# brunothg/sfm-mvs-pipeline

Measured on AMD Instinct MI355X. Metric: descriptor-pairs/s matched, higher is better.
Workload: dtype int8->int32 (exact; f32 in/out); 1 GPU; 50 images x 8192 SIFT-128 f32, unordered all-pairs (1225 pairs); descriptors_per_image=8192, pairs=1225, parallelism=pair-sharded x1

## Files before the change

sfm-mvs-pipeline_amd/csrc/match_kernels.hip:

```cpp
#include <hip/hip_runtime.h>
#include <cstdint>
#include <climits>
#include <cstdlib>
#include "match_common.hpp"
#include "diag.hpp"
#include "sift_fp6.hpp"

namespace sfmx {

typedef int i32x4 __attribute__((ext_vector_type(4)));
typedef int i32x16 __attribute__((ext_vector_type(16)));
typedef unsigned u32x4 __attribute__((ext_vector_type(4)));
typedef int i32x8 __attribute__((ext_vector_type(8)));
typedef float f32x4 __attribute__((ext_vector_type(4)));
typedef float f32x16 __attribute__((ext_vector_type(16)));

#define GLOBAL_AS __attribute__((address_space(1)))
#define LDS_AS __attribute__((address_space(3)))

__device__ __forceinline__ int med3i(int a, int b, int c) { return max(min(a, b), min(max(a, b), c)); }
__device__ __forceinline__ int v_med3(int a, int b, int c) {
    int d;
    asm("v_med3_i32 %0, %1, %2, %3" : "=v"(d) : "v"(a), "v"(b), "v"(c));
    return d;
// ... 688 lines not shown
template <bool CERT>
__device__ __forceinline__ void screen6_forward(float k1, float k2, int r1, int qi, int nt, int2 q2, int emax2, int amax2,
                                                double ratio, int pair, int64_t dense_base, int32_t* __restrict__ qlist,
                                                int32_t* __restrict__ qcount, int32_t* __restrict__ qmask,
                                                unsigned long long* __restrict__ top2, int32_t* __restrict__ qlist2,
                                                int32_t* __restrict__ qcount2) {
    const int usable = (int)(nt >= 2) & (int)(k2 > fp6::KEY_VALID);
    const int rej = usable & fp6::certainly_rejected(k1, k2, q2.x, q2.y, emax2, amax2, ratio);
    if (rej == 0) {
        const int64_t slot = dense_base + atomicAdd(&qcount[pair], 1);
        qlist[slot] = qi;
        if constexpr (CERT) {
            const int cert = fp6::certified(k1, k2, r1, nt, q2.x, q2.y, emax2, amax2, ratio);
            qmask[slot] = cert ? 1 << r1 : QMASK_FULL_ROUTE;
            if (!cert) qlist2[dense_base + atomicAdd(&qcount2[pair], 1)] = (int32_t)(slot - dense_base);
        } else {
            qmask[slot] = 0xFFFF;
        }
        top2[2 * slot] = ~0ull;
        top2[2 * slot + 1] = ~0ull;
    }
}

template <int QT, int WAVES, int MINW, int STAGE, bool CERT>
__global__ __launch_bounds__(WAVES * 64, MINW)
void sift_screen6_kernel(const WorkItem* __restrict__ work, const PairDev* __restrict__ pairs,
                         const ImgDev* __restrict__ imgs, const uint32_t* __restrict__ desc6,
                         const float* __restrict__ keyf, const int2* __restrict__ ne,
                         const int32_t* __restrict__ imax,
                         int32_t* __restrict__ qlist, int32_t* __restrict__ qcount, double ratio,
                         int32_t* __restrict__ qmask, unsigned long long* __restrict__ top2,
                         int32_t* __restrict__ qlist2, int32_t* __restrict__ qcount2) {
    static_assert(QT * WAVES * 16 == 512, "work items are 512 queries");
    static_assert(WAVES == 4 && STAGE % 128 == 0 && ROW_ALIGN % STAGE == 0, "whole DMA instructions per wave; stages inside the padded rows");
    constexpr int A_BYTES = STAGE * 64, B_BYTES = STAGE * 32;
    constexpr int GA = A_BYTES / (WAVES * 64 * 16), GB = B_BYTES / (WAVES * 64 * 16), GK = STAGE / 64;
    constexpr int BUF_BYTES = A_BYTES + B_BYTES + STAGE * 4;
    __shared__ __attribute__((aligned(16))) char lds[2 * BUF_BYTES];

    const int wid = threadIdx.x >> 6, lane = threadIdx.x & 63, g = lane >> 4, l16 = lane & 15;
    const WorkItem w = work[xcd_remap(blockIdx.x, gridDim.x)];
    const PairDev P = pairs[w.pair];
    const ImgDev L = imgs[P.left], R = imgs[P.right];
    const int nq = L.rows, nt = R.rows;
    const int qbase = w.q0 + wid * (QT * 16);

    i32x8 bq[QT];
#pragma unroll
    for (int qt = 0; qt < QT; ++qt) {
        const uint32_t* src = desc6 + (L.row0 + qbase + qt * 16 + l16) * fp6::ROW_WORDS;
        const i32x4 lo = *reinterpret_cast<const i32x4*>(src + 4 * g);
        const int2 hi = *reinterpret_cast<const int2*>(src + 16 + 2 * g);
        bq[qt] = i32x8{lo.x, lo.y, lo.z, lo.w, hi.x, hi.y, 0, 0};
    }
    float ch[QT][4];
#pragma unroll
    for (int qt = 0; qt < QT; ++qt)
#pragma unroll
        for (int i = 0; i < 4; ++i) ch[qt][i] = fp6::KEY_INIT;

    const int nstages = (nt + STAGE - 1) / STAGE;
    const char* tbase = reinterpret_cast<const char*>(desc6 + R.row0 * fp6::ROW_WORDS);
    const float* kbase = keyf + R.row0;
    auto stage = [&](int s, int buf) {
        char* base = lds + buf * BUF_BYTES;
#pragma unroll
        for (int i = 0; i < GA; ++i) {
            const int p = i * WAVES * 64 + threadIdx.x;
            const int rr = p >> 2, c = (p & 3) ^ fp6::swz_a(rr);
            const char* gp = tbase + (int64_t)(s * STAGE + rr) * fp6::ROW_BYTES + 16 * c;
            __builtin_amdgcn_global_load_lds((const GLOBAL_AS void*)gp,
                                             (LDS_AS void*)(base + (i * WAVES + wid) * 1024), 16, 0, 0);
        }
#pragma unroll
        for (int i = 0; i < GB; ++i) {
            const int p = i * WAVES * 64 + threadIdx.x;
            const int rr = p >> 1, c = (p & 1) ^ fp6::swz_b(rr);
            const char* gp = tbase + (int64_t)(s * STAGE + rr) * fp6::ROW_BYTES + 64 + 16 * c;
            __builtin_amdgcn_global_load_lds((const GLOBAL_AS void*)gp,
                                             (LDS_AS void*)(base + A_BYTES + (i * WAVES + wid) * 1024), 16, 0, 0);
        }
        if (wid < GK)
            __builtin_amdgcn_global_load_lds((const GLOBAL_AS void*)(kbase + s * STAGE + wid * 64 + lane),
                                             (LDS_AS void*)(base + A_BYTES + B_BYTES + wid * 256), 4, 0, 0);
    };

    if (nstages > 0) stage(0, 0);
    asm volatile("s_waitcnt vmcnt(0)" ::: "memory");
    __syncthreads();
    for (int s = 0; s < nstages; ++s) {
        const int buf = s & 1;
        if (s + 1 < nstages) stage(s + 1, buf ^ 1);
        const char* base = lds + buf * BUF_BYTES;
#pragma unroll
        for (int t = 0; t < STAGE / 32; ++t) {
            i32x8 a[2];
            f32x4 cinit[2];
#pragma unroll
            for (int b = 0; b < 2; ++b) {
                const int row = t * 32 + b * 16 + l16;
                const i32x4 lo = *reinterpret_cast<const i32x4*>(base + row * 64 + 16 * (g ^ fp6::swz_a(row)));
                const int2 hi = *reinterpret_cast<const int2*>(base + A_BYTES + row * 32 +
                                                               16 * ((g >> 1) ^ fp6::swz_b(row)) + 8 * (g & 1));
                a[b] = i32x8{lo.x, lo.y, lo.z, lo.w, hi.x, hi.y, 0, 0};
                cinit[b] = *reinterpret_cast<const f32x4*>(base + A_BYTES + B_BYTES + 4 * (t * 32 + b * 16 + 4 * g));
            }
#pragma unroll
            for (int qt = 0; qt < QT; ++qt) {
                const f32x4 acc0 = __builtin_amdgcn_mfma_scale_f32_16x16x128_f8f6f4(a[0], bq[qt], cinit[0], 2, 2, 0, 0x7f7f7f7f,
                                                                                    0, 0x7f7f7f7f);
                const f32x4 acc1 = __builtin_amdgcn_mfma_scale_f32_16x16x128_f8f6f4(a[1], bq[qt], cinit[1], 2, 2, 0, 0x7f7f7f7f,
                                                                                    0, 0x7f7f7f7f);
#pragma unroll
                for (int i = 0; i < 4; ++i) ch[qt][i] = fmaxf(fmaxf(ch[qt][i], acc0[i]), acc1[i]);
            }
        }
        asm volatile("s_waitcnt vmcnt(0)" ::: "memory");
        __syncthreads();
    }

    const int emax2 = imax[2 * P.right], amax2 = imax[2 * P.right + 1];
    static_assert(QT % 4 == 0, "four tiles per decision pass");
    float kk1[4] = {}, kk2[4] = {};
    int rr1[4] = {};
#pragma unroll
    for (int qt = 0; qt < QT; ++qt) {
        float k1 = fp6::KEY_INIT, k2 = fp6::KEY_INIT;
        int r1 = 4 * g;
#pragma unroll
        for (int i = 0; i < 4; ++i) {
            const float v = ch[qt][i];
            if constexpr (CERT) r1 = v > k1 ? 4 * g + i : r1;
            k2 = fmaxf(k2, fminf(k1, v));
            k1 = fmaxf(k1, v);
        }
// ... 14 lines not shown
        for (int j = 1; j < 4; ++j) {
            k1 = g == j ? kk1[j] : k1;
            k2 = g == j ? kk2[j] : k2;
            r1 = g == j ? rr1[j] : r1;
        }
        const int qi = qbase + ((qt & ~3) + g) * 16 + l16;
        if (qi >= nq || nt == 0) continue;
        screen6_forward<CERT>(k1, k2, r1, qi, nt, ne[L.row0 + qi], emax2, amax2, ratio, w.pair, P.dense_base, qlist, qcount,
                              qmask, top2, qlist2, qcount2);
    }
}

template <int WAVES, int MINW, int STAGE, bool CERT>
__global__ __launch_bounds__(WAVES * 64, MINW)
void sift_screen6w_kernel(const WorkItem* __restrict__ work, const PairDev* __restrict__ pairs,
                          const ImgDev* __restrict__ imgs, const uint32_t* __restrict__ desc6,
                          const float* __restrict__ keyf, const int2* __restrict__ ne,
                          const int32_t* __restrict__ imax,
                          int32_t* __restrict__ qlist, int32_t* __restrict__ qcount, double ratio,
                          int32_t* __restrict__ qmask, unsigned long long* __restrict__ top2,
                          int32_t* __restrict__ qlist2, int32_t* __restrict__ qcount2) {
    constexpr int QT = 4;
    static_assert(QT * WAVES * 32 == 512, "work items are 512 queries");
    static_assert(WAVES == 4 && STAGE % 128 == 0 && ROW_ALIGN % STAGE == 0, "whole DMA instructions per wave; stages inside the padded rows");
    constexpr int A_BYTES = STAGE * 64, B_BYTES = STAGE * 32;
    constexpr int GA = A_BYTES / (WAVES * 64 * 16), GB = B_BYTES / (WAVES * 64 * 16), GK = STAGE / 64;
    constexpr int BUF_BYTES = A_BYTES + B_BYTES + STAGE * 4;
    __shared__ __attribute__((aligned(16))) char lds[2 * BUF_BYTES];

    const int wid = threadIdx.x >> 6, lane = threadIdx.x & 63, h = lane >> 5, l32 = lane & 31;
    const WorkItem w = work[xcd_remap(blockIdx.x, gridDim.x)];
    const PairDev P = pairs[w.pair];
    const ImgDev L = imgs[P.left], R = imgs[P.right];
    const int nq = L.rows, nt = R.rows;
    const int qbase = w.q0 + wid * (QT * 32);

    i32x8 bq[QT][2];
#pragma unroll
    for (int qt = 0; qt < QT; ++qt) {
        const uint32_t* src = desc6 + (L.row0 + qbase + qt * 32 + l32) * fp6::ROW_WORDS;
#pragma unroll
        for (int m = 0; m < 2; ++m) {
            const int f = fp6::frag32(m, h);
            const i32x4 lo = *reinterpret_cast<const i32x4*>(src + fp6::word_index(f, 0));
            const int2 hi = *reinterpret_cast<const int2*>(src + fp6::word_index(f, 4));
            bq[qt][m] = i32x8{lo.x, lo.y, lo.z, lo.w, hi.x, hi.y, 0, 0};
        }
    }
    float ch[QT][8];
#pragma unroll
    for (int qt = 0; qt < QT; ++qt)
#pragma unroll
        for (int c = 0; c < 8; ++c) ch[qt][c] = fp6::KEY_INIT;

    const int nstages = (nt + STAGE - 1) / STAGE;
    const char* tbase = reinterpret_cast<const char*>(desc6 + R.row0 * fp6::ROW_WORDS);
    const float* kbase = keyf + R.row0;
    auto stage = [&](int s, int buf) {
        char* base = lds + buf * BUF_BYTES;
#pragma unroll
        for (int i = 0; i < GA; ++i) {
            const int p = i * WAVES * 64 + threadIdx.x;
            const int rr = p >> 2, c = (p & 3) ^ fp6::swz_a(rr);
            const char* gp = tbase + (int64_t)(s * STAGE + rr) * fp6::ROW_BYTES + 16 * c;
            __builtin_amdgcn_global_load_lds((const GLOBAL_AS void*)gp,
                                             (LDS_AS void*)(base + (i * WAVES + wid) * 1024), 16, 0, 0);
        }
#pragma unroll
        for (int i = 0; i < GB; ++i) {
            const int p = i * WAVES * 64 + threadIdx.x;
            const int rr = p >> 1, c = (p & 1) ^ fp6::swz_b(rr);
            const char* gp = tbase + (int64_t)(s * STAGE + rr) * fp6::ROW_BYTES + 64 + 16 * c;
            __builtin_amdgcn_global_load_lds((const GLOBAL_AS void*)gp,
                                             (LDS_AS void*)(base + A_BYTES + (i * WAVES + wid) * 1024), 16, 0, 0);
        }
        if (wid < GK)
            __builtin_amdgcn_global_load_lds((const GLOBAL_AS void*)(kbase + s * STAGE + wid * 64 + lane),
                                             (LDS_AS void*)(base + A_BYTES + B_BYTES + wid * 256), 4, 0, 0);
    };

    if (nstages > 0) stage(0, 0);
    asm volatile("s_waitcnt vmcnt(0)" ::: "memory");
    __syncthreads();
    for (int s = 0; s < nstages; ++s) {
        const int buf = s & 1;
        if (s + 1 < nstages) stage(s + 1, buf ^ 1);
        const char* base = lds + buf * BUF_BYTES;
#pragma unroll
        for (int t = 0; t < STAGE / 32; ++t) {
            i32x8 a[2];
            f32x16 key;
#pragma unroll
            for (int m = 0; m < 2; ++m) {
                const int f = fp6::frag32(m, h), row = t * 32 + l32;
                const i32x4 lo = *reinterpret_cast<const i32x4*>(base + fp6::lds_a32(row, f));
                const int2 hi = *reinterpret_cast<const int2*>(base + fp6::lds_b32(STAGE, row, f));
                a[m] = i32x8{lo.x, lo.y, lo.z, lo.w, hi.x, hi.y, 0, 0};
            }
#pragma unroll
            for (int k = 0; k < 4; ++k) {
                const f32x4 kv = *reinterpret_cast<const f32x4*>(base + fp6::lds_key32(STAGE, t * 32, k, h));
                key[4 * k + 0] = kv.x; key[4 * k + 1] = kv.y; key[4 * k + 2] = kv.z; key[4 * k + 3] = kv.w;
            }
#pragma unroll
            for (int qt = 0; qt < QT; ++qt) {
                f32x16 acc = __builtin_amdgcn_mfma_scale_f32_32x32x64_f8f6f4(a[0], bq[qt][0], key, 2, 2, 0, 0x7f7f7f7f, 0,
                                                                             0x7f7f7f7f);
                acc = __builtin_amdgcn_mfma_scale_f32_32x32x64_f8f6f4(a[1], bq[qt][1], acc, 2, 2, 0, 0x7f7f7f7f, 0, 0x7f7f7f7f);
#pragma unroll
                for (int c = 0; c < 8; ++c) ch[qt][c] = fmaxf(fmaxf(ch[qt][c], acc[c]), acc[c + 8]);
            }
        }
        asm volatile("s_waitcnt vmcnt(0)" ::: "memory");
        __syncthreads();
    }

    const int emax2 = imax[2 * P.right], amax2 = imax[2 * P.right + 1];
    float kk1[2] = {}, kk2[2] = {};
    int rr1[2] = {};
#pragma unroll
    for (int qt = 0; qt < QT; ++qt) {
        float k1 = fp6::KEY_INIT, k2 = fp6::KEY_INIT;
        int r1 = fp6::chain_subset32(0, h);
#pragma unroll
        for (int c = 0; c < 8; ++c) {
            const float v = ch[qt][c];
            if constexpr (CERT) r1 = v > k1 ? fp6::chain_subset32(c, h) : r1;
            k2 = fmaxf(k2, fminf(k1, v));
            k1 = fmaxf(k1, v);
        }
        {
// ... 215 lines not shown
}
#endif
hipError_t launch_prep_l2_batch(const PrepImg* tab, int n, int max_rows_pad, int8_t* desc8, int32_t* norm,
                                int32_t* keyc, int32_t* keyc2, int32_t* flags, uint32_t* desc6, float* keyf,
                                int2* ne, int32_t* imax, hipStream_t st) {
    if (n == 0 || max_rows_pad == 0) return hipSuccess;
    prep_l2_batch_kernel<<<dim3((unsigned)((max_rows_pad + PREP_ROWS - 1) / PREP_ROWS), (unsigned)n), 256, 0, st>>>(
        tab, desc8, norm, keyc, keyc2, flags, Fp6Rows{desc6, keyf, ne}, imax);
    return hipGetLastError();
}
__global__ __launch_bounds__(256)
void publish_flags_kernel(const int32_t* __restrict__ flags, int n, int32_t* __restrict__ dst, unsigned* __restrict__ seq,
                          unsigned v) {
    for (int i = threadIdx.x; i < n; i += blockDim.x) dst[i] = flags[i];
    __threadfence_system();
    __syncthreads();
    if (threadIdx.x == 0) __hip_atomic_store(seq, v, __ATOMIC_RELEASE, __HIP_MEMORY_SCOPE_SYSTEM);
}
hipError_t launch_publish_flags(const int32_t* flags, int n, int32_t* dst, unsigned* seq, unsigned v, hipStream_t st) {
    publish_flags_kernel<<<1, 256, 0, st>>>(flags, n, dst, seq, v);
    return hipGetLastError();
}
#ifdef SFMX_DIAG
hipError_t launch_probe_xor80(int8_t* p, int64_t bytes, hipStream_t st) {
    const int64_t n = bytes / 4;
    if (n == 0) return hipSuccess;
    probe_xor80_kernel<<<(unsigned)((n + 255) / 256), 256, 0, st>>>(reinterpret_cast<uint32_t*>(p), n);
    return hipGetLastError();
}
#endif

template <int ISH>
__global__ __launch_bounds__(1024)
void compact_work_kernel(const int32_t* __restrict__ porder, int n_pairs, const int32_t* __restrict__ qcount,
                         WorkItem* __restrict__ work2, int32_t* __restrict__ work2_n, int ride = 0) {
    __shared__ int wsum[16];
    const int tid = threadIdx.x, lane = tid & 63, wv = tid >> 6;
    const int per = (n_pairs + 1023) / 1024, p0 = min(tid * per, n_pairs), p1 = min(p0 + per, n_pairs);
    int mine = 0;
    auto items = [&](int c) { return c > ride ? (c + (1 << ISH) - 1) >> ISH : 0; };
    for (int i = p0; i < p1; ++i) mine += items(qcount[porder[i]]);
    int incl = mine;
    for (int o = 1; o < 64; o <<= 1) {
        const int v = __shfl_up(incl, o);
        if (lane >= o) incl += v;
    }
// ... 180 lines not shown

    for (int s = 0; s < nstages; ++s) {
        const int buf = s & 1;
        if (s + 1 < nstages) stage(s + 1, buf ^ 1);
        const char* base = lds + buf * BUF_BYTES;
#pragma unroll
        for (int t = 0; t < STAGE / 32; ++t) {
            const int row = t * 32 + l32;
            i32x4 a[4];
#pragma unroll
            for (int m = 0; m < 4; ++m) {
                const int slot = (2 * m + h) ^ ((row >> 1) & 7);
                a[m] = *reinterpret_cast<const i32x4*>(base + row * ROWB + 16 * slot);
            }
            f32x16 cinit;
#pragma unroll
            for (int g = 0; g < 4; ++g) {
                const f32x4 kv = *reinterpret_cast<const f32x4*>(base + DESC_BYTES + 4 * (t * 32 + 8 * g + 4 * h));
                cinit[4 * g + 0] = kv.x; cinit[4 * g + 1] = kv.y; cinit[4 * g + 2] = kv.z; cinit[4 * g + 3] = kv.w;
            }
            f32x16 acc[QT];
#pragma unroll
            for (int qt = 0; qt < QT; ++qt) {
                acc[qt] = __builtin_amdgcn_mfma_scale_f32_32x32x64_f8f6f4(i8of(a[0]), i8of(bq[qt][0]), cinit, 4, 4, 0,
                                                                          0x7f7f7f7f, 0, 0x7f7f7f7f);
#pragma unroll
                for (int m = 1; m < 4; ++m)
                    acc[qt] = __builtin_amdgcn_mfma_scale_f32_32x32x64_f8f6f4(i8of(a[m]), i8of(bq[qt][m]), acc[qt], 4, 4,
                                                                              0, 0x7f7f7f7f, 0, 0x7f7f7f7f);
            }
#pragma unroll
            for (int qt = 0; qt < QT; ++qt) select(acc[qt], c1[qt], c2[qt]);
        }
        if ((s % SPC) == SPC - 1 || s + 1 == nstages) {
            const int cb = (s / SPC) * CHUNK;
#pragma unroll
            for (int qt = 0; qt < QT; ++qt) {
                const float p1 = __shfl_xor(c1[qt], 32), p2 = __shfl_xor(c2[qt], 32);
                const float m1 = fmaxf(c1[qt], p1), m2 = fmaxf(fminf(c1[qt], p1), fmaxf(c2[qt], p2));
#pragma unroll
                for (int e = 0; e < 2; ++e) {
                    const float v = e == 0 ? m1 : m2;
                    if (v >= KEY_FLOOR) {
                        const float ip = __builtin_floorf(v);
                        const int dot = (int)ip - 767;
                        const int t_ = (256 - dot) >> 1;
                        const int j_ = cb + 16383 - (int)((v - ip) * 16384.0f);
                        if (t_ < T2[qt]) {
                            if (t_ < T1[qt]) { T2[qt] = T1[qt]; J2[qt] = J1[qt]; T1[qt] = t_; J1[qt] = j_; }
                            else { T2[qt] = t_; J2[qt] = j_; }
                        }
                    }
// ... 94 lines not shown
    for (int s = 0; s < nstages; ++s) {
        const int buf = s & 1;
        if (s + 1 < nstages) stage(s + 1, buf ^ 1);
        const char* base = lds + buf * BUF_BYTES;
#pragma unroll
        for (int t = 0; t < STAGE / 32; ++t) {
            i32x4 a[2][2];
            f32x4 cinit[2];
#pragma unroll
            for (int b = 0; b < 2; ++b) {
                const int row = t * 32 + b * 16 + l16;
#pragma unroll
                for (int m = 0; m < 2; ++m) {
                    const int slot = (4 * m + g) ^ ((row >> 1) & 7);
                    a[b][m] = *reinterpret_cast<const i32x4*>(base + row * ROWB + 16 * slot);
                }
                cinit[b] = *reinterpret_cast<const f32x4*>(base + DESC_BYTES + 4 * (t * 32 + b * 16 + 4 * g));
            }
#pragma unroll
            for (int qt = 0; qt < QT; ++qt) {
                f32x4 acc[2];
#pragma unroll
                for (int b = 0; b < 2; ++b) {
                    acc[b] = __builtin_amdgcn_mfma_scale_f32_16x16x128_f8f6f4(i8of(a[b][0]), i8of(bq[qt][0]), cinit[b], 4, 4,
                                                                              0, 0x7f7f7f7f, 0, 0x7f7f7f7f);
                    acc[b] = __builtin_amdgcn_mfma_scale_f32_16x16x128_f8f6f4(i8of(a[b][1]), i8of(bq[qt][1]), acc[b], 4, 4,
                                                                              0, 0x7f7f7f7f, 0, 0x7f7f7f7f);
                }
#pragma unroll
                for (int b = 0; b < 2; ++b)
#pragma unroll
                    for (int r = 0; r < 4; r += 2) {
                        const float ka = acc[b][r], kb = acc[b][r + 1];
                        c2[qt] = fmaxf(__builtin_amdgcn_fmed3f(c1[qt], ka, kb), c2[qt]);
                        c1[qt] = fmaxf(c1[qt], fmaxf(ka, kb));
                    }
            }
        }
        if ((s % SPC) == SPC - 1 || s + 1 == nstages) {
            const int cb = (s / SPC) * CHUNK;
#pragma unroll
            for (int qt = 0; qt < QT; ++qt) {
                float m1 = c1[qt], m2 = c2[qt];
#pragma unroll
                for (int o = 16; o <= 32; o <<= 1) {
                    const float p1 = __shfl_xor(m1, o), p2 = __shfl_xor(m2, o);
                    m2 = fmaxf(fminf(m1, p1), fmaxf(m2, p2));
                    m1 = fmaxf(m1, p1);
                }
#pragma unroll
// ... 103 lines not shown
    for (int s = 0; s < nstages; ++s) {
        const int buf = s & 1;
        if (s + 1 < nstages) stage(s + 1, buf ^ 1);
        const char* base = lds + buf * BUF_BYTES;
#pragma unroll
        for (int t = 0; t < STAGE / 32; ++t) {
            i32x4 a[2][2];
            f32x4 cinit[2];
#pragma unroll
            for (int b = 0; b < 2; ++b) {
                const int row = t * 32 + b * 16 + l16;
#pragma unroll
                for (int m = 0; m < 2; ++m) {
                    const int slot = (4 * m + g) ^ ((row >> 1) & 7);
                    a[b][m] = *reinterpret_cast<const i32x4*>(base + row * ROWB + 16 * slot);
                }
                cinit[b] = *reinterpret_cast<const f32x4*>(base + DESC_BYTES + 4 * (t * 32 + b * 16 + 4 * g));
            }
#pragma unroll
            for (int qt = 0; qt < QT; ++qt) {
                f32x4 acc[2];
#pragma unroll
                for (int b = 0; b < 2; ++b) {
                    acc[b] = __builtin_amdgcn_mfma_scale_f32_16x16x128_f8f6f4(i8of(a[b][0]), i8of(bq[qt][0]), cinit[b], 4, 4,
                                                                              0, 0x7f7f7f7f, 0, 0x7f7f7f7f);
                    acc[b] = __builtin_amdgcn_mfma_scale_f32_16x16x128_f8f6f4(i8of(a[b][1]), i8of(bq[qt][1]), acc[b], 4, 4,
                                                                              0, 0x7f7f7f7f, 0, 0x7f7f7f7f);
                }
#pragma unroll
                for (int i = 0; i < 4; ++i) ch[qt][i] = fmaxf(fmaxf(ch[qt][i], acc[0][i]), acc[1][i]);
            }
        }
        asm volatile("s_waitcnt vmcnt(0)" ::: "memory");
        __syncthreads();
    }

#pragma unroll
    for (int qt = 0; qt < QT; ++qt) {
        float k1 = 0.f, k2 = 0.f;
#pragma unroll
        for (int i = 0; i < 4; ++i) {
            const float v = ch[qt][i];
            k2 = fmaxf(k2, fminf(k1, v));
            k1 = fmaxf(k1, v);
        }
#pragma unroll
        for (int o = 16; o <= 32; o <<= 1) {
            const float p1 = __shfl_xor(k1, o), p2 = __shfl_xor(k2, o);
            k2 = fmaxf(fminf(k1, p1), fmaxf(k2, p2));
            k1 = fmaxf(k1, p1);
// ... 107 lines not shown
                    keys_lds[i] = (i < rows && j < nt) ? (float)(767 * 16384 + 16383 - li) * (1.0f / 16384.0f) : 0.f;
                }
                asm volatile("s_waitcnt vmcnt(0)" ::: "memory");
                __syncthreads();
                if (active) {
                    for (int t = 0; t < rows / 32; ++t) {
                        i32x4 a[2][2];
                        f32x4 cinit[2];
#pragma unroll
                        for (int b = 0; b < 2; ++b) {
                            const int row = t * 32 + b * 16 + l16;
#pragma unroll
                            for (int m = 0; m < 2; ++m) {
                                const int slot = (4 * m + g) ^ ((row >> 1) & 7);
                                a[b][m] = *reinterpret_cast<const i32x4*>(rows_lds + row * ROWB + 16 * slot);
                            }
                            cinit[b] = *reinterpret_cast<const f32x4*>(keys_lds + t * 32 + b * 16 + 4 * g);
                        }
#pragma unroll
                        for (int qt = 0; qt < QT; ++qt) {
                            f32x4 acc[2];
#pragma unroll
                            for (int b = 0; b < 2; ++b) {
                                acc[b] = __builtin_amdgcn_mfma_scale_f32_16x16x128_f8f6f4(i8of(a[b][0]), i8of(bq[qt][0]), cinit[b],
                                                                                          4, 4, 0, 0x7f7f7f7f, 0, 0x7f7f7f7f);
                                acc[b] = __builtin_amdgcn_mfma_scale_f32_16x16x128_f8f6f4(i8of(a[b][1]), i8of(bq[qt][1]), acc[b],
                                                                                          4, 4, 0, 0x7f7f7f7f, 0, 0x7f7f7f7f);
                            }
#pragma unroll
                            for (int b = 0; b < 2; ++b)
#pragma unroll
                                for (int q = 0; q < 4; q += 2) {
                                    const float ka = acc[b][q], kb = acc[b][q + 1];
                                    c2[qt] = fmaxf(__builtin_amdgcn_fmed3f(c1[qt], ka, kb), c2[qt]);
                                    c1[qt] = fmaxf(c1[qt], fmaxf(ka, kb));
                                }
                        }
                    }
                }
            }
            if (active) {
#pragma unroll
                for (int qt = 0; qt < QT; ++qt) {
                    float m1 = c1[qt], m2 = c2[qt];
#pragma unroll
                    for (int o = 16; o <= 32; o <<= 1) {
                        const float p1 = __shfl_xor(m1, o), p2 = __shfl_xor(m2, o);
                        m2 = fmaxf(fminf(m1, p1), fmaxf(m2, p2));
                        m1 = fmaxf(m1, p1);
                    }
// ... 786 lines not shown
```

sfm-mvs-pipeline_amd/csrc/matcher.cpp:

```cpp
#include <hip/hip_runtime.h>
#include "diag.hpp"
#include <algorithm>
#include <atomic>
#include <cstdio>
#include <cstdlib>
#include <cstring>
#include <mutex>
#include <numeric>
#include <string>
#include <thread>
#include <vector>

#include "../../include/sfmx.h"
#include "match_common.hpp"
#include "sift_fp6.hpp"

namespace sfmx {
hipError_t launch_prep_l2(const float*, int, int, int, int8_t*, int32_t*, int32_t*, int32_t*, int32_t*, hipStream_t);
hipError_t launch_probe_xor80(int8_t*, int64_t, hipStream_t);
hipError_t launch_publish_flags(const int32_t*, int, int32_t*, unsigned*, unsigned, hipStream_t);
hipError_t launch_prep_l2_batch(const PrepImg*, int, int, int8_t*, int32_t*, int32_t*, int32_t*, int32_t*, uint32_t*, float*,
                                int2*, int32_t*, hipStream_t);
hipError_t launch_prep_f32(const float*, int, int, int, float*, hipStream_t);
hipError_t launch_prep_hamming(const uint8_t*, int, int, int, uint8_t*, hipStream_t);
hipError_t launch_sift_knn2(const WorkItem*, int, const PairDev*, const ImgDev*, const int8_t*, const int32_t*,
                            const int32_t*, const int32_t*, int32_t*, int32_t*, int, const int32_t*, WorkItem*,
                            int32_t*, int32_t*, float*, int2*, int32_t*, double, hipStream_t, hipEvent_t, int32_t*,
                            unsigned long long*, unsigned long long*, bool, const uint32_t*, const float*, const int2*,
                            const int32_t*);
hipError_t launch_finish_lists(const PairRec*, int, const int32_t*, const int32_t*, const int32_t*, unsigned long long*,
                               const unsigned long long*, int2*, int32_t*, const int8_t*, const int32_t*, const int32_t*,
                               const float*, double, int, int, int, int, int64_t*, int32_t*, int64_t*, DMatchDev*, int32_t*,
                               hipStream_t, hipEvent_t);
bool persist_screens();
hipError_t launch_sift_slow(const int2*, const int32_t*, const PairDev*, const ImgDev*, const int8_t*,
                            const int32_t*, int32_t*, float*, double, hipStream_t);
hipError_t launch_sift_f32(const WorkItem*, int, const PairDev*, const ImgDev*, const float*, int32_t*, float*,
                           double, hipStream_t);
hipError_t launch_orb_knn2(const WorkItem*, int, const PairDev*, const ImgDev*, const uint8_t*, int32_t*, float*,
                           double, hipStream_t);
hipError_t launch_prep_hamming_fp4(const uint8_t*, int, int, int, uint8_t*, int32_t*, hipStream_t);
hipError_t launch_orb_mfma(const WorkItem*, int, const PairDev*, const ImgDev*, const uint8_t*, const int32_t*,
// ... 759 lines not shown
    for (int p = 0; p < m->n_pairs; ++p) { a += h[p]; b += h[arena_qcount2(m->n_pairs) + p]; }
    if (forwarded) *forwarded = a;
    if (full_route) *full_route = b;
    return SFMX_OK;
}
int sfmx_diag_matcher_prep_rows(sfmx_matcher* m, int img, uint32_t* desc6, float* keyf, int32_t* ne, int32_t* norm,
                                int32_t* imax) {
    if (!m) return fail(SFMX_EINVAL, "null matcher");
    if (m->norm != SFMX_NORM_L2 || img < 0 || img >= m->n_imgs) return fail(SFMX_EINVAL, "no such L2 image");
    DeviceGuard g(m->device);
    if (hipDeviceSynchronize() != hipSuccess) return fail(SFMX_EINTERNAL, "device synchronize failed");
    const ImgDev& d = m->imgs[img];
    const size_t n = (size_t)d.rows_pad;
    hipError_t e = hipSuccess;
    if (desc6 && e == hipSuccess)
        e = hipMemcpy(desc6, m->desc6.as<uint32_t>() + d.row0 * fp6::ROW_WORDS, n * fp6::ROW_BYTES, hipMemcpyDeviceToHost);
    if (keyf && e == hipSuccess) e = hipMemcpy(keyf, m->keyf.as<float>() + d.row0, n * 4, hipMemcpyDeviceToHost);
    if (ne && e == hipSuccess) e = hipMemcpy(ne, m->ne.as<int2>() + d.row0, n * sizeof(int2), hipMemcpyDeviceToHost);
    if (norm && e == hipSuccess) e = hipMemcpy(norm, m->normv.as<int32_t>() + d.row0, n * 4, hipMemcpyDeviceToHost);
    if (imax && e == hipSuccess) e = hipMemcpy(imax, m->imax.as<int32_t>() + 2 * img, 8, hipMemcpyDeviceToHost);
    if (e != hipSuccess) return fail(SFMX_EINTERNAL, hipGetErrorString(e));
    return d.rows_pad;
}
#endif

int sfmx_matcher_timing(sfmx_matcher* m, float* main_kernel_ms, float* total_ms) {
    if (!m) return fail(SFMX_EINVAL, "null matcher");
    if (!m->ev_recorded) return fail(SFMX_ESTATE, "no timing before run");
    DeviceGuard g(m->device);
    HIPCHK(hipEventSynchronize(m->ev[2]));
    float a = 0.f, b = 0.f;
    HIPCHK(hipEventElapsedTime(&a, m->ev[0], m->ev[1]));
    HIPCHK(hipEventElapsedTime(&b, m->ev[0], m->ev[2]));
    if (main_kernel_ms) *main_kernel_ms = a;
    if (total_ms) *total_ms = b;
    return SFMX_OK;
}

int sfmx_matcher_timing_history(sfmx_matcher* m, float* main_kernel_ms, float* screen_ms, int32_t n) {
    if (!m) return fail(SFMX_EINVAL, "null matcher");
    if (!m->ev_recorded) return fail(SFMX_ESTATE, "no timing before run");
    if (n < 0) return fail(SFMX_EINVAL, "negative count");
    DeviceGuard g(m->device);
    HIPCHK(hipEventSynchronize(m->ev[2]));
    const long long k = std::min<long long>({(long long)n, m->runs, (long long)sfmx_matcher::EV_RING});
    for (long long i = 0; i < k; ++i) {
// ... 107 lines not shown
```

sfm-mvs-pipeline_amd/csrc/sift_fp6.hpp:

```cpp
#pragma once
#include <cstdint>

#if defined(__HIPCC__) || defined(__CUDACC__)
#define SFMX_FP6_HD __host__ __device__ __forceinline__
#else
#define SFMX_FP6_HD inline
#endif

namespace sfmx {
namespace fp6 {

constexpr int OFFSET = 32;
constexpr int SCALE = 4;
constexpr int ROW_BYTES = 96;
constexpr int ROW_WORDS = 24;
constexpr float PAD_KEY = -1.0e30f;
constexpr float KEY_VALID = -1.0e29f;
constexpr float KEY_INIT = -3.0e38f;
constexpr double SLACK = 1025.0;

SFMX_FP6_HD int quant_m(int a) {
    const int mag = a < 0 ? -a : a, s = (mag >> 6) < 2 ? (mag >> 6) : 2;
    const int m = ((mag + (2 << s)) >> (2 + s)) << s;
    return a < 0 ? -m : m;
// ... 12 lines not shown

inline void pack_row(const unsigned* codes , uint32_t* out ) {
    for (int i = 0; i < ROW_WORDS; ++i) out[i] = 0;
    for (int k = 0; k < 128; ++k) {
        const int g = k >> 5, bit = 6 * (k & 31);
        const uint64_t v = (uint64_t)(codes[k] & 63u) << (bit & 31);
        out[word_index(g, bit >> 5)] |= (uint32_t)v;
        if ((bit & 31) > 26) out[word_index(g, (bit >> 5) + 1)] |= (uint32_t)(v >> 32);
    }
}

SFMX_FP6_HD constexpr int swz_a(int row) { return (0 - (row >> 2)) & 3; }
SFMX_FP6_HD constexpr int swz_b(int row) { return (row >> 3) & 1; }

SFMX_FP6_HD constexpr int frag32(int m, int h) { return 2 * m + h; }
SFMX_FP6_HD constexpr int acc_row32(int i, int h) { return (i & 3) + 8 * (i >> 2) + 4 * h; }
SFMX_FP6_HD constexpr int chain_subset32(int c, int h) { return (c & 3) + 4 * h + 8 * (c >> 2); }
SFMX_FP6_HD constexpr int lds_a32(int row, int f) { return row * 64 + 16 * (f ^ swz_a(row)); }
SFMX_FP6_HD constexpr int lds_b32(int stage, int row, int f) {
    return stage * 64 + row * 32 + 16 * ((f >> 1) ^ swz_b(row)) + 8 * (f & 1);
}
SFMX_FP6_HD constexpr int lds_key32(int stage, int row0, int k, int h) { return stage * 96 + 4 * (row0 + 8 * k + 4 * h); }

SFMX_FP6_HD float sqrt_rn(int64_t s) { return (float)__builtin_sqrt((double)s); }

SFMX_FP6_HD int certainly_rejected(float k1, float k2, int na, int e2q, int emax2, int amax2, double ratio) {
    const double E = __builtin_sqrt((double)na * (double)emax2) +
                     __builtin_sqrt((double)e2q) * (__builtin_sqrt((double)amax2) + __builtin_sqrt((double)emax2));
    const double M = E + SLACK;
    double lo = (double)na - 2.0 * ((double)k1 * 1024.0 + M);
    double hi = (double)na - 2.0 * ((double)k2 * 1024.0 - M);
    lo = lo < 0.0 ? 0.0 : lo;
    hi = hi < 0.0 ? 0.0 : (hi > 1.0e12 ? 1.0e12 : hi);
    lo = lo > 1.0e12 ? 1.0e12 : lo;
    const int64_t s1 = (int64_t)__builtin_floor(lo), s2 = (int64_t)__builtin_ceil(hi);
    return (int)!((double)sqrt_rn(s1) < (double)sqrt_rn(s2) * ratio);
}

constexpr int64_t SQRT_SAFE_S = 1 << 22;
SFMX_FP6_HD int certified(float k1, float k2, int r1, int nt, int na, int e2q, int emax2, int amax2, double ratio) {
    const double E = __builtin_sqrt((double)na * (double)emax2) +
                     __builtin_sqrt((double)e2q) * (__builtin_sqrt((double)amax2) + __builtin_sqrt((double)emax2));
    const double M = E + SLACK;
    double s1 = (double)na - 2.0 * ((double)k1 * 1024.0 - M);
    double lo = (double)na - 2.0 * ((double)k2 * 1024.0 + M);
    double hi = (double)na - 2.0 * ((double)k2 * 1024.0 - M);
// ... 12 lines not shown
```

Measured before the change: 17230 billion descriptor-pairs/s.

## Use buffer-resource LDS DMA, hoisted LDS read addresses, and unscaled MFMA form

Moves the stage loader into a helper that builds buffer resource descriptors once and issues buffer_load_lds with precomputed per-thread voffsets and scalar row offsets. This replaces per-iteration 64-bit global address arithmetic. The FP6 screen kernel hoists its swizzled LDS read pointers out of the loop, relying on the swizzle having a 16-row period. All scaled-MFMA calls now go through wrappers whose scale operands are zero (the plain non-scaled MFMA form) instead of 0x7f7f7f7f. A diagnostic kernel is added to check that the two forms give the same results, and the volatile 64-bit LDS read may constrain scheduling.

```diff
diff --git a/sfm-mvs-pipeline_amd/csrc/match_kernels.hip b/sfm-mvs-pipeline_amd/csrc/match_kernels.hip
--- a/sfm-mvs-pipeline_amd/csrc/match_kernels.hip
+++ b/sfm-mvs-pipeline_amd/csrc/match_kernels.hip
@@ -734,6 +734,45 @@
     }
 }
 
+template <int STAGE>
+struct Screen6Stage {
+    static constexpr int WAVES = 4;
+    static constexpr int A_BYTES = STAGE * 64, B_BYTES = STAGE * 32;
+    static constexpr int GA = A_BYTES / (WAVES * 64 * 16), GB = B_BYTES / (WAVES * 64 * 16), GK = STAGE / 64;
+    static constexpr int BUF_BYTES = A_BYTES + B_BYTES + STAGE * 4;
+    static_assert(STAGE % 128 == 0 && ROW_ALIGN % STAGE == 0, "whole DMA instructions per wave; stages inside the padded rows");
+    __amdgpu_buffer_rsrc_t rows, keys;
+    int va, vb, vk;
+    int wid;
+
+    __device__ __forceinline__ Screen6Stage(const uint32_t* __restrict__ desc6, const float* __restrict__ keyf, const ImgDev& R) {
+        const int tid = threadIdx.x;
+        wid = __builtin_amdgcn_readfirstlane(tid >> 6);
+        const int ra = tid >> 2, rb = tid >> 1;
+        va = ra * fp6::ROW_BYTES + 16 * ((tid & 3) ^ fp6::swz_a(ra));
+        vb = rb * fp6::ROW_BYTES + 64 + 16 * ((tid & 1) ^ fp6::swz_b(rb));
+        vk = (tid & 63) * 4;
+        rows = __builtin_amdgcn_make_buffer_rsrc(const_cast<uint32_t*>(desc6 + R.row0 * fp6::ROW_WORDS), 0,
+                                                 R.rows_pad * fp6::ROW_BYTES, 0x00020000);
+        keys = __builtin_amdgcn_make_buffer_rsrc(const_cast<float*>(keyf + R.row0), 0, R.rows_pad * 4, 0x00020000);
+    }
+    __device__ __forceinline__ void issue(char* lds, int s, int buf) const {
+        char* base = lds + buf * BUF_BYTES;
+        const int row0 = s * STAGE;
+#pragma unroll
+        for (int i = 0; i < GA; ++i)
+            __builtin_amdgcn_raw_ptr_buffer_load_lds(rows, (LDS_AS void*)(base + (i * WAVES + wid) * 1024), 16, va,
+                                                     (row0 + i * 64) * fp6::ROW_BYTES, 0, 0);
+#pragma unroll
+        for (int i = 0; i < GB; ++i)
+            __builtin_amdgcn_raw_ptr_buffer_load_lds(rows, (LDS_AS void*)(base + A_BYTES + (i * WAVES + wid) * 1024), 16, vb,
+                                                     (row0 + i * 128) * fp6::ROW_BYTES, 0, 0);
+        if (wid < GK)
+            __builtin_amdgcn_raw_ptr_buffer_load_lds(keys, (LDS_AS void*)(base + A_BYTES + B_BYTES + wid * 256), 4, vk,
+                                                     (row0 + wid * 64) * 4, 0, 0);
+    }
+};
+
 template <int QT, int WAVES, int MINW, int STAGE, bool CERT>
 __global__ __launch_bounds__(WAVES * 64, MINW)
 void sift_screen6_kernel(const WorkItem* __restrict__ work, const PairDev* __restrict__ pairs,
@@ -744,17 +783,18 @@
                          int32_t* __restrict__ qmask, unsigned long long* __restrict__ top2,
                          int32_t* __restrict__ qlist2, int32_t* __restrict__ qcount2) {
     static_assert(QT * WAVES * 16 == 512, "work items are 512 queries");
-    static_assert(WAVES == 4 && STAGE % 128 == 0 && ROW_ALIGN % STAGE == 0, "whole DMA instructions per wave; stages inside the padded rows");
-    constexpr int A_BYTES = STAGE * 64, B_BYTES = STAGE * 32;
-    constexpr int GA = A_BYTES / (WAVES * 64 * 16), GB = B_BYTES / (WAVES * 64 * 16), GK = STAGE / 64;
-    constexpr int BUF_BYTES = A_BYTES + B_BYTES + STAGE * 4;
+    using Stage = Screen6Stage<STAGE>;
+    static_assert(WAVES == Stage::WAVES, "whole DMA instructions per wave");
+    constexpr int A_BYTES = Stage::A_BYTES, B_BYTES = Stage::B_BYTES, BUF_BYTES = Stage::BUF_BYTES;
     __shared__ __attribute__((aligned(16))) char lds[2 * BUF_BYTES];
 
-    const int wid = threadIdx.x >> 6, lane = threadIdx.x & 63, g = lane >> 4, l16 = lane & 15;
+    const int lane = threadIdx.x & 63, g = lane >> 4, l16 = lane & 15;
     const WorkItem w = work[xcd_remap(blockIdx.x, gridDim.x)];
     const PairDev P = pairs[w.pair];
     const ImgDev L = imgs[P.left], R = imgs[P.right];
     const int nq = L.rows, nt = R.rows;
+    const Stage stager(desc6, keyf, R);
+    const int wid = stager.wid;
     const int qbase = w.q0 + wid * (QT * 16);
 
     i32x8 bq[QT];
@@ -772,57 +812,34 @@
         for (int i = 0; i < 4; ++i) ch[qt][i] = fp6::KEY_INIT;
 
     const int nstages = (nt + STAGE - 1) / STAGE;
-    const char* tbase = reinterpret_cast<const char*>(desc6 + R.row0 * fp6::ROW_WORDS);
-    const float* kbase = keyf + R.row0;
-    auto stage = [&](int s, int buf) {
-        char* base = lds + buf * BUF_BYTES;
-#pragma unroll
-        for (int i = 0; i < GA; ++i) {
-            const int p = i * WAVES * 64 + threadIdx.x;
-            const int rr = p >> 2, c = (p & 3) ^ fp6::swz_a(rr);
-            const char* gp = tbase + (int64_t)(s * STAGE + rr) * fp6::ROW_BYTES + 16 * c;
-            __builtin_amdgcn_global_load_lds((const GLOBAL_AS void*)gp,
-                                             (LDS_AS void*)(base + (i * WAVES + wid) * 1024), 16, 0, 0);
-        }
-#pragma unroll
-        for (int i = 0; i < GB; ++i) {
-            const int p = i * WAVES * 64 + threadIdx.x;
-            const int rr = p >> 1, c = (p & 1) ^ fp6::swz_b(rr);
-            const char* gp = tbase + (int64_t)(s * STAGE + rr) * fp6::ROW_BYTES + 64 + 16 * c;
-            __builtin_amdgcn_global_load_lds((const GLOBAL_AS void*)gp,
-                                             (LDS_AS void*)(base + A_BYTES + (i * WAVES + wid) * 1024), 16, 0, 0);
-        }
-        if (wid < GK)
-            __builtin_amdgcn_global_load_lds((const GLOBAL_AS void*)(kbase + s * STAGE + wid * 64 + lane),
-                                             (LDS_AS void*)(base + A_BYTES + B_BYTES + wid * 256), 4, 0, 0);
-    };
-
-    if (nstages > 0) stage(0, 0);
+    const char* ra = lds + l16 * 64 + 16 * (g ^ fp6::swz_a(l16));
+    const char* rb = lds + A_BYTES + l16 * 32 + 16 * ((g >> 1) ^ fp6::swz_b(l16)) + 8 * (g & 1);
+    const char* rk = lds + A_BYTES + B_BYTES + 16 * g;
+    static_assert(fp6::swz_a(16) == fp6::swz_a(0) && fp6::swz_b(16) == fp6::swz_b(0), "swizzle period of 16 rows");
+
+    if (nstages > 0) stager.issue(lds, 0, 0);
     asm volatile("s_waitcnt vmcnt(0)" ::: "memory");
     __syncthreads();
     for (int s = 0; s < nstages; ++s) {
         const int buf = s & 1;
-        if (s + 1 < nstages) stage(s + 1, buf ^ 1);
-        const char* base = lds + buf * BUF_BYTES;
+        if (s + 1 < nstages) stager.issue(lds, s + 1, buf ^ 1);
+        const char *pa = ra + buf * BUF_BYTES, *pb = rb + buf * BUF_BYTES, *pk = rk + buf * BUF_BYTES;
 #pragma unroll
         for (int t = 0; t < STAGE / 32; ++t) {
             i32x8 a[2];
             f32x4 cinit[2];
 #pragma unroll
             for (int b = 0; b < 2; ++b) {
-                const int row = t * 32 + b * 16 + l16;
-                const i32x4 lo = *reinterpret_cast<const i32x4*>(base + row * 64 + 16 * (g ^ fp6::swz_a(row)));
-                const int2 hi = *reinterpret_cast<const int2*>(base + A_BYTES + row * 32 +
-                                                               16 * ((g >> 1) ^ fp6::swz_b(row)) + 8 * (g & 1));
-                a[b] = i32x8{lo.x, lo.y, lo.z, lo.w, hi.x, hi.y, 0, 0};
-                cinit[b] = *reinterpret_cast<const f32x4*>(base + A_BYTES + B_BYTES + 4 * (t * 32 + b * 16 + 4 * g));
+                const int blk = 2 * t + b;
+                const i32x4 lo = *reinterpret_cast<const i32x4*>(pa + blk * 16 * 64);
+                const long long hi = *(const volatile LDS_AS long long*)(pb + blk * 16 * 32);
+                a[b] = i32x8{lo.x, lo.y, lo.z, lo.w, (int)hi, (int)(hi >> 32), 0, 0};
+                cinit[b] = *reinterpret_cast<const f32x4*>(pk + blk * 16 * 4);
             }
 #pragma unroll
             for (int qt = 0; qt < QT; ++qt) {
-                const f32x4 acc0 = __builtin_amdgcn_mfma_scale_f32_16x16x128_f8f6f4(a[0], bq[qt], cinit[0], 2, 2, 0, 0x7f7f7f7f,
-                                                                                    0, 0x7f7f7f7f);
-                const f32x4 acc1 = __builtin_amdgcn_mfma_scale_f32_16x16x128_f8f6f4(a[1], bq[qt], cinit[1], 2, 2, 0, 0x7f7f7f7f,
-                                                                                    0, 0x7f7f7f7f);
+                const f32x4 acc0 = fp6::mfma16<fp6::FMT_E2M3, false>(a[0], bq[qt], cinit[0]);
+                const f32x4 acc1 = fp6::mfma16<fp6::FMT_E2M3, false>(a[1], bq[qt], cinit[1]);
 #pragma unroll
                 for (int i = 0; i < 4; ++i) ch[qt][i] = fmaxf(fmaxf(ch[qt][i], acc0[i]), acc1[i]);
             }
@@ -883,17 +900,18 @@
                           int32_t* __restrict__ qlist2, int32_t* __restrict__ qcount2) {
     constexpr int QT = 4;
     static_assert(QT * WAVES * 32 == 512, "work items are 512 queries");
-    static_assert(WAVES == 4 && STAGE % 128 == 0 && ROW_ALIGN % STAGE == 0, "whole DMA instructions per wave; stages inside the padded rows");
-    constexpr int A_BYTES = STAGE * 64, B_BYTES = STAGE * 32;
-    constexpr int GA = A_BYTES / (WAVES * 64 * 16), GB = B_BYTES / (WAVES * 64 * 16), GK = STAGE / 64;
-    constexpr int BUF_BYTES = A_BYTES + B_BYTES + STAGE * 4;
+    using Stage = Screen6Stage<STAGE>;
+    static_assert(WAVES == Stage::WAVES, "whole DMA instructions per wave");
+    constexpr int BUF_BYTES = Stage::BUF_BYTES;
     __shared__ __attribute__((aligned(16))) char lds[2 * BUF_BYTES];
 
-    const int wid = threadIdx.x >> 6, lane = threadIdx.x & 63, h = lane >> 5, l32 = lane & 31;
+    const int lane = threadIdx.x & 63, h = lane >> 5, l32 = lane & 31;
     const WorkItem w = work[xcd_remap(blockIdx.x, gridDim.x)];
     const PairDev P = pairs[w.pair];
     const ImgDev L = imgs[P.left], R = imgs[P.right];
     const int nq = L.rows, nt = R.rows;
+    const Stage stager(desc6, keyf, R);
+    const int wid = stager.wid;
     const int qbase = w.q0 + wid * (QT * 32);
 
     i32x8 bq[QT][2];
@@ -915,37 +933,12 @@
         for (int c = 0; c < 8; ++c) ch[qt][c] = fp6::KEY_INIT;
 
     const int nstages = (nt + STAGE - 1) / STAGE;
-    const char* tbase = reinterpret_cast<const char*>(desc6 + R.row0 * fp6::ROW_WORDS);
-    const float* kbase = keyf + R.row0;
-    auto stage = [&](int s, int buf) {
-        char* base = lds + buf * BUF_BYTES;
-#pragma unroll
-        for (int i = 0; i < GA; ++i) {
-            const int p = i * WAVES * 64 + threadIdx.x;
-            const int rr = p >> 2, c = (p & 3) ^ fp6::swz_a(rr);
-            const char* gp = tbase + (int64_t)(s * STAGE + rr) * fp6::ROW_BYTES + 16 * c;
-            __builtin_amdgcn_global_load_lds((const GLOBAL_AS void*)gp,
-                                             (LDS_AS void*)(base + (i * WAVES + wid) * 1024), 16, 0, 0);
-        }
-#pragma unroll
-        for (int i = 0; i < GB; ++i) {
-            const int p = i * WAVES * 64 + threadIdx.x;
-            const int rr = p >> 1, c = (p & 1) ^ fp6::swz_b(rr);
-            const char* gp = tbase + (int64_t)(s * STAGE + rr) * fp6::ROW_BYTES + 64 + 16 * c;
-            __builtin_amdgcn_global_load_lds((const GLOBAL_AS void*)gp,
-                                             (LDS_AS void*)(base + A_BYTES + (i * WAVES + wid) * 1024), 16, 0, 0);
-        }
-        if (wid < GK)
-            __builtin_amdgcn_global_load_lds((const GLOBAL_AS void*)(kbase + s * STAGE + wid * 64 + lane),
-                                             (LDS_AS void*)(base + A_BYTES + B_BYTES + wid * 256), 4, 0, 0);
-    };
-
-    if (nstages > 0) stage(0, 0);
+    if (nstages > 0) stager.issue(lds, 0, 0);
     asm volatile("s_waitcnt vmcnt(0)" ::: "memory");
     __syncthreads();
     for (int s = 0; s < nstages; ++s) {
         const int buf = s & 1;
-        if (s + 1 < nstages) stage(s + 1, buf ^ 1);
+        if (s + 1 < nstages) stager.issue(lds, s + 1, buf ^ 1);
         const char* base = lds + buf * BUF_BYTES;
 #pragma unroll
         for (int t = 0; t < STAGE / 32; ++t) {
@@ -965,9 +958,8 @@
             }
 #pragma unroll
             for (int qt = 0; qt < QT; ++qt) {
-                f32x16 acc = __builtin_amdgcn_mfma_scale_f32_32x32x64_f8f6f4(a[0], bq[qt][0], key, 2, 2, 0, 0x7f7f7f7f, 0,
-                                                                             0x7f7f7f7f);
-                acc = __builtin_amdgcn_mfma_scale_f32_32x32x64_f8f6f4(a[1], bq[qt][1], acc, 2, 2, 0, 0x7f7f7f7f, 0, 0x7f7f7f7f);
+                f32x16 acc = fp6::mfma32<fp6::FMT_E2M3, false>(a[0], bq[qt][0], key);
+                acc = fp6::mfma32<fp6::FMT_E2M3, false>(a[1], bq[qt][1], acc);
 #pragma unroll
                 for (int c = 0; c < 8; ++c) ch[qt][c] = fmaxf(fmaxf(ch[qt][c], acc[c]), acc[c + 8]);
             }
@@ -1229,6 +1221,40 @@
     return hipGetLastError();
 }
 #ifdef SFMX_DIAG
+template <int FMT>
+__global__ __launch_bounds__(64)
+void mfma_forms16_kernel(const i32x8* __restrict__ a, const i32x8* __restrict__ b, const f32x4* __restrict__ c,
+                         f32x4* __restrict__ d_scaled, f32x4* __restrict__ d_unscaled) {
+    const int64_t i = (int64_t)blockIdx.x * 64 + threadIdx.x;
+    d_scaled[i] = fp6::mfma16<FMT, true>(a[i], b[i], c[i]);
+    d_unscaled[i] = fp6::mfma16<FMT, false>(a[i], b[i], c[i]);
+}
+template <int FMT>
+__global__ __launch_bounds__(64)
+void mfma_forms32_kernel(const i32x8* __restrict__ a, const i32x8* __restrict__ b, const f32x16* __restrict__ c,
+                         f32x16* __restrict__ d_scaled, f32x16* __restrict__ d_unscaled) {
+    const int64_t i = (int64_t)blockIdx.x * 64 + threadIdx.x, j = (int64_t)blockIdx.x * 128 + threadIdx.x;
+    d_scaled[i] = fp6::mfma32<FMT, true>(a[j + 64], b[j + 64], fp6::mfma32<FMT, true>(a[j], b[j], c[i]));
+    d_unscaled[i] = fp6::mfma32<FMT, false>(a[j + 64], b[j + 64], fp6::mfma32<FMT, false>(a[j], b[j], c[i]));
+}
+hipError_t launch_mfma_forms(int shape, int fmt, int n, const int32_t* a, const int32_t* b, const float* c, float* d_scaled,
+                             float* d_unscaled, hipStream_t st) {
+    if (n <= 0) return hipSuccess;
+    if ((shape != 16 && shape != 32) || (fmt != fp6::FMT_E2M3 && fmt != fp6::FMT_E2M1)) return hipErrorInvalidValue;
+    const i32x8 *pa = reinterpret_cast<const i32x8*>(a), *pb = reinterpret_cast<const i32x8*>(b);
+    if (shape == 16) {
+        const f32x4* pc = reinterpret_cast<const f32x4*>(c);
+        f32x4 *ds = reinterpret_cast<f32x4*>(d_scaled), *du = reinterpret_cast<f32x4*>(d_unscaled);
+        if (fmt == fp6::FMT_E2M3) mfma_forms16_kernel<fp6::FMT_E2M3><<<n, 64, 0, st>>>(pa, pb, pc, ds, du);
+        else mfma_forms16_kernel<fp6::FMT_E2M1><<<n, 64, 0, st>>>(pa, pb, pc, ds, du);
+    } else {
+        const f32x16* pc = reinterpret_cast<const f32x16*>(c);
+        f32x16 *ds = reinterpret_cast<f32x16*>(d_scaled), *du = reinterpret_cast<f32x16*>(d_unscaled);
+        if (fmt == fp6::FMT_E2M3) mfma_forms32_kernel<fp6::FMT_E2M3><<<n, 64, 0, st>>>(pa, pb, pc, ds, du);
+        else mfma_forms32_kernel<fp6::FMT_E2M1><<<n, 64, 0, st>>>(pa, pb, pc, ds, du);
+    }
+    return hipGetLastError();
+}
 hipError_t launch_probe_xor80(int8_t* p, int64_t bytes, hipStream_t st) {
     const int64_t n = bytes / 4;
     if (n == 0) return hipSuccess;
@@ -1455,12 +1481,10 @@
             f32x16 acc[QT];
 #pragma unroll
             for (int qt = 0; qt < QT; ++qt) {
-                acc[qt] = __builtin_amdgcn_mfma_scale_f32_32x32x64_f8f6f4(i8of(a[0]), i8of(bq[qt][0]), cinit, 4, 4, 0,
-                                                                          0x7f7f7f7f, 0, 0x7f7f7f7f);
+                acc[qt] = fp6::mfma32<fp6::FMT_E2M1, false>(i8of(a[0]), i8of(bq[qt][0]), cinit);
 #pragma unroll
                 for (int m = 1; m < 4; ++m)
-                    acc[qt] = __builtin_amdgcn_mfma_scale_f32_32x32x64_f8f6f4(i8of(a[m]), i8of(bq[qt][m]), acc[qt], 4, 4,
-                                                                              0, 0x7f7f7f7f, 0, 0x7f7f7f7f);
+                    acc[qt] = fp6::mfma32<fp6::FMT_E2M1, false>(i8of(a[m]), i8of(bq[qt][m]), acc[qt]);
             }
 #pragma unroll
             for (int qt = 0; qt < QT; ++qt) select(acc[qt], c1[qt], c2[qt]);
@@ -1601,10 +1625,8 @@
                 f32x4 acc[2];
 #pragma unroll
                 for (int b = 0; b < 2; ++b) {
-                    acc[b] = __builtin_amdgcn_mfma_scale_f32_16x16x128_f8f6f4(i8of(a[b][0]), i8of(bq[qt][0]), cinit[b], 4, 4,
-                                                                              0, 0x7f7f7f7f, 0, 0x7f7f7f7f);
-                    acc[b] = __builtin_amdgcn_mfma_scale_f32_16x16x128_f8f6f4(i8of(a[b][1]), i8of(bq[qt][1]), acc[b], 4, 4,
-                                                                              0, 0x7f7f7f7f, 0, 0x7f7f7f7f);
+                    acc[b] = fp6::mfma16<fp6::FMT_E2M1, false>(i8of(a[b][0]), i8of(bq[qt][0]), cinit[b]);
+                    acc[b] = fp6::mfma16<fp6::FMT_E2M1, false>(i8of(a[b][1]), i8of(bq[qt][1]), acc[b]);
                 }
 #pragma unroll
                 for (int b = 0; b < 2; ++b)
@@ -1754,10 +1776,8 @@
                 f32x4 acc[2];
 #pragma unroll
                 for (int b = 0; b < 2; ++b) {
-                    acc[b] = __builtin_amdgcn_mfma_scale_f32_16x16x128_f8f6f4(i8of(a[b][0]), i8of(bq[qt][0]), cinit[b], 4, 4,
-                                                                              0, 0x7f7f7f7f, 0, 0x7f7f7f7f);
-                    acc[b] = __builtin_amdgcn_mfma_scale_f32_16x16x128_f8f6f4(i8of(a[b][1]), i8of(bq[qt][1]), acc[b], 4, 4,
-                                                                              0, 0x7f7f7f7f, 0, 0x7f7f7f7f);
+                    acc[b] = fp6::mfma16<fp6::FMT_E2M1, false>(i8of(a[b][0]), i8of(bq[qt][0]), cinit[b]);
+                    acc[b] = fp6::mfma16<fp6::FMT_E2M1, false>(i8of(a[b][1]), i8of(bq[qt][1]), acc[b]);
                 }
 #pragma unroll
                 for (int i = 0; i < 4; ++i) ch[qt][i] = fmaxf(fmaxf(ch[qt][i], acc[0][i]), acc[1][i]);
@@ -1911,10 +1931,8 @@
                             f32x4 acc[2];
 #pragma unroll
                             for (int b = 0; b < 2; ++b) {
-                                acc[b] = __builtin_amdgcn_mfma_scale_f32_16x16x128_f8f6f4(i8of(a[b][0]), i8of(bq[qt][0]), cinit[b],
-                                                                                          4, 4, 0, 0x7f7f7f7f, 0, 0x7f7f7f7f);
-                                acc[b] = __builtin_amdgcn_mfma_scale_f32_16x16x128_f8f6f4(i8of(a[b][1]), i8of(bq[qt][1]), acc[b],
-                                                                                          4, 4, 0, 0x7f7f7f7f, 0, 0x7f7f7f7f);
+                                acc[b] = fp6::mfma16<fp6::FMT_E2M1, false>(i8of(a[b][0]), i8of(bq[qt][0]), cinit[b]);
+                                acc[b] = fp6::mfma16<fp6::FMT_E2M1, false>(i8of(a[b][1]), i8of(bq[qt][1]), acc[b]);
                             }
 #pragma unroll
                             for (int b = 0; b < 2; ++b)
diff --git a/sfm-mvs-pipeline_amd/csrc/matcher.cpp b/sfm-mvs-pipeline_amd/csrc/matcher.cpp
--- a/sfm-mvs-pipeline_amd/csrc/matcher.cpp
+++ b/sfm-mvs-pipeline_amd/csrc/matcher.cpp
@@ -18,6 +18,7 @@
 namespace sfmx {
 hipError_t launch_prep_l2(const float*, int, int, int, int8_t*, int32_t*, int32_t*, int32_t*, int32_t*, hipStream_t);
 hipError_t launch_probe_xor80(int8_t*, int64_t, hipStream_t);
+hipError_t launch_mfma_forms(int, int, int, const int32_t*, const int32_t*, const float*, float*, float*, hipStream_t);
 hipError_t launch_publish_flags(const int32_t*, int, int32_t*, unsigned*, unsigned, hipStream_t);
 hipError_t launch_prep_l2_batch(const PrepImg*, int, int, int8_t*, int32_t*, int32_t*, int32_t*, int32_t*, uint32_t*, float*,
                                 int2*, int32_t*, hipStream_t);
@@ -823,6 +824,48 @@
     if (e != hipSuccess) return fail(SFMX_EINTERNAL, hipGetErrorString(e));
     return d.rows_pad;
 }
+int sfmx_diag_matcher_prep_rows8(sfmx_matcher* m, int img, int8_t* desc8, int32_t* keyc, int32_t* keyc2) {
+    if (!m) return fail(SFMX_EINVAL, "null matcher");
+    if (m->norm != SFMX_NORM_L2 || img < 0 || img >= m->n_imgs) return fail(SFMX_EINVAL, "no such L2 image");
+    DeviceGuard g(m->device);
+    if (hipDeviceSynchronize() != hipSuccess) return fail(SFMX_EINTERNAL, "device synchronize failed");
+    const ImgDev& d = m->imgs[img];
+    const size_t n = (size_t)d.rows_pad;
+    hipError_t e = hipSuccess;
+    if (desc8 && e == hipSuccess)
+        e = hipMemcpy(desc8, m->desc8.as<int8_t>() + d.row0 * SIFT_DIM, n * SIFT_DIM, hipMemcpyDeviceToHost);
+    if (keyc && e == hipSuccess) e = hipMemcpy(keyc, m->keyc.as<int32_t>() + d.row0, n * 4, hipMemcpyDeviceToHost);
+    if (keyc2 && e == hipSuccess) e = hipMemcpy(keyc2, m->keyc2.as<int32_t>() + d.row0, n * 4, hipMemcpyDeviceToHost);
+    if (e != hipSuccess) return fail(SFMX_EINTERNAL, hipGetErrorString(e));
+    return d.rows_pad;
+}
+int sfmx_diag_mfma_forms(int device, int shape, int fmt, int n, const int32_t* a, const int32_t* b, const float* c,
+                         float* d_scaled, float* d_unscaled) {
+    if (n < 0 || (shape != 16 && shape != 32) || (fmt != 2 && fmt != 4) || !a || !b || !c || !d_scaled || !d_unscaled)
+        return fail(SFMX_EINVAL, "mfma forms: shape 16 | 32, fmt 2 | 4, no null array");
+    if (n == 0) return SFMX_OK;
+    DeviceGuard g(device);
+    const size_t ab = (size_t)n * (shape == 16 ? 1 : 2) * 64 * 8 * 4, cd = (size_t)n * 64 * (shape == 16 ? 4 : 16) * 4;
+    DevBuf da, db, dc, ds, du;
+    auto run = [&]() -> int {
+        for (DevBuf* buf : {&da, &db})
+            if (const int rc = buf->ensure(ab)) return rc;
+        for (DevBuf* buf : {&dc, &ds, &du})
+            if (const int rc = buf->ensure(cd)) return rc;
+        HIPCHK(hipMemcpy(da.p, a, ab, hipMemcpyHostToDevice));
+        HIPCHK(hipMemcpy(db.p, b, ab, hipMemcpyHostToDevice));
+        HIPCHK(hipMemcpy(dc.p, c, cd, hipMemcpyHostToDevice));
+        HIPCHK(launch_mfma_forms(shape, fmt, n, da.as<int32_t>(), db.as<int32_t>(), dc.as<float>(), ds.as<float>(),
+                                 du.as<float>(), nullptr));
+        HIPCHK(hipDeviceSynchronize());
+        HIPCHK(hipMemcpy(d_scaled, ds.p, cd, hipMemcpyDeviceToHost));
+        HIPCHK(hipMemcpy(d_unscaled, du.p, cd, hipMemcpyDeviceToHost));
+        return SFMX_OK;
+    };
+    const int rc = run();
+    for (DevBuf* buf : {&da, &db, &dc, &ds, &du}) buf->release();
+    return rc;
+}
 #endif
 
 int sfmx_matcher_timing(sfmx_matcher* m, float* main_kernel_ms, float* total_ms) {
diff --git a/sfm-mvs-pipeline_amd/csrc/sift_fp6.hpp b/sfm-mvs-pipeline_amd/csrc/sift_fp6.hpp
--- a/sfm-mvs-pipeline_amd/csrc/sift_fp6.hpp
+++ b/sfm-mvs-pipeline_amd/csrc/sift_fp6.hpp
@@ -58,6 +58,23 @@
 }
 SFMX_FP6_HD constexpr int lds_key32(int stage, int row0, int k, int h) { return stage * 96 + 4 * (row0 + 8 * k + 4 * h); }
 
+#if defined(__HIPCC__)
+constexpr int FMT_E2M3 = 2, FMT_E2M1 = 4;
+typedef int mfma_i32x8 __attribute__((ext_vector_type(8)));
+typedef float mfma_f32x4 __attribute__((ext_vector_type(4)));
+typedef float mfma_f32x16 __attribute__((ext_vector_type(16)));
+template <int FMT, bool SCALED>
+__device__ __forceinline__ mfma_f32x4 mfma16(mfma_i32x8 a, mfma_i32x8 b, mfma_f32x4 c) {
+    if constexpr (SCALED) return __builtin_amdgcn_mfma_scale_f32_16x16x128_f8f6f4(a, b, c, FMT, FMT, 0, 0x7f7f7f7f, 0, 0x7f7f7f7f);
+    else return __builtin_amdgcn_mfma_scale_f32_16x16x128_f8f6f4(a, b, c, FMT, FMT, 0, 0, 0, 0);
+}
+template <int FMT, bool SCALED>
+__device__ __forceinline__ mfma_f32x16 mfma32(mfma_i32x8 a, mfma_i32x8 b, mfma_f32x16 c) {
+    if constexpr (SCALED) return __builtin_amdgcn_mfma_scale_f32_32x32x64_f8f6f4(a, b, c, FMT, FMT, 0, 0x7f7f7f7f, 0, 0x7f7f7f7f);
+    else return __builtin_amdgcn_mfma_scale_f32_32x32x64_f8f6f4(a, b, c, FMT, FMT, 0, 0, 0, 0);
+}
+#endif
+
 SFMX_FP6_HD float sqrt_rn(int64_t s) { return (float)__builtin_sqrt((double)s); }
 
 SFMX_FP6_HD int certainly_rejected(float k1, float k2, int na, int e2q, int emax2, int amax2, double ratio) {
```

Measured after the change: 19230 billion descriptor-pairs/s, median of 6. 11.6% higher.
